# sydney-machine-learning/parallel-tempering-neural-net

Measured on AMD Instinct MI355X. Metric: MCMC samples/sec (all replicas) + swap-accept rate; Sunspot 64-replica FNN, higher is better.
Workload: dtype f32

## Files before the change

### parallel-tempering-neural-net_amd/csrc/ptnn_dev_pack.hpp

```cpp

constexpr int PK_WAVES = 8, PK_SWEEP_WAVES = 2, PK_FWD_WAVES = 4;
__host__ __device__ constexpr int pack_slots(int nred) { return PK_SWEEP_WAVES * (WAVE >> nred); }

__host__ __device__ inline size_t pack_slot_floats(int PS) { return 2 * (size_t)PS; }
__host__ __device__ inline size_t pack_ring_floats(int PS, int nslots) { return (size_t)2 * nslots * ((size_t)PS + 4); }
__host__ __device__ inline size_t pack_lds_floats(int Nall, int IPY, int PS, int H, int FWS, int nslots) {
    return (size_t)(Nall + 2) * IPY + 4 * (size_t)PS + MAX_WAVES * 8 + (size_t)nslots * SL_COUNT +
           (size_t)nslots * pack_slot_floats(PS) + pack_ring_floats(PS, nslots) + (size_t)PK_WAVES * fw_floats(H, FWS);
}
constexpr int PK_MULTI_MAXG = 4;
__host__ __device__ inline size_t pack_multi_lds_floats(int Nall, int IPY, int PS, int H, int FWS, int nslots) {
    return pack_lds_floats(Nall, IPY, PS, H, FWS, nslots) + pack_ring_floats(PS, (PK_MULTI_MAXG - 1) * nslots) + 2 * (size_t)PS + SL_COUNT + 8;
}

template <int TASK, int I, int O, int PK_NRED, bool MULTI = false>
__device__ __forceinline__ void segment_pack_body(const SegParams& p, const SegDyn& dyn, const int step_begin, const int n_steps) {
    constexpr int PK_NG = WAVE >> PK_NRED, PK_SLOTS = pack_slots(PK_NRED);
    extern __shared__ __attribute__((aligned(16))) float smem[];
    const int G = MULTI ? p.G : 1;
    const int lb = MULTI ? xcd_block(G) : (int)blockIdx.x;
    const int r = MULTI ? lb / G : lb, grp = MULTI ? lb - r * G : 0;
    const int KT = G * PK_SLOTS, s0 = grp * PK_SLOTS;
    const int gid = p.first_global + r;
    const int tid = threadIdx.x, nthr = blockDim.x;
    const int wave = tid >> 6, lane = tid & 63;
    const int Nall = p.Ntr + p.Nte;
    const int P = p.P, PS = p.PS, H = p.H;
    float* q = smem;
    float* xy = q; q += (Nall + 2) * p.IPY;
    float* w_cur = q; q += PS;
    float* w_gd = q; q += PS;
    float* rec_w = q; q += PS;
    float* rec_alt = q; q += PS;
    float* red = q; q += MAX_WAVES * 8;
    float* slots = q; q += PK_SLOTS * SL_COUNT;
    const size_t SLF = pack_slot_floats(PS);
    float* sl0 = q; q += PK_SLOTS * SLF;
    constexpr int RING = (MULTI ? 2 * PK_MULTI_MAXG : 2) * PK_SLOTS;
    float* ring_n = q; q += (size_t)RING * PS;
    float* ring_s = q; q += (size_t)RING * 4;
    float* my_fw = q + (size_t)wave * fw_floats(H, p.FWS);
    q += (size_t)PK_WAVES * fw_floats(H, p.FWS);
    float* win_v = q; q += MULTI ? 2 * (size_t)PS : 0;
    float* win_s = q; q += MULTI ? SL_COUNT : 0;
    float* gverd = q;
    granule_t* const xv = MULTI ? p.xverdict + (size_t)r * 2 * MAX_SLOTS : nullptr;
    granule_t* const xsl = MULTI ? p.xslots + (size_t)r * 2 * MAX_SLOTS * SL_COUNT : nullptr;
    granule_t* const xwv = MULTI ? p.xw + (size_t)r * 2 * G * 2 * PS : nullptr;
    unsigned epoch = dyn.epoch_base;
    int xpar = 0;
    bool failed = false;
    auto s_prop = [&](int s_) { return sl0 + (size_t)s_ * SLF; };
    auto s_pgd = [&](int s_) { return sl0 + (size_t)s_ * SLF + PS; };

    {
        const float4* src = reinterpret_cast<const float4*>(p.data);
        float4* dst = reinterpret_cast<float4*>(xy);
        for (int e = tid; e < ((Nall + 2) * p.IPY) >> 2; e += nthr) dst[e] = src[e];
    }
    float* gw = dyn.w_state + (size_t)r * PS;
    for (int j = tid; j < PS; j += nthr) {
        w_cur[j] = gw[j];
        rec_w[j] = p.rec_w[(size_t)r * PS + j];
        w_gd[j] = dyn.gd_w[(size_t)r * PS + j];
    }
    __syncthreads();

    const float T = uni_f(p.temps[r]);
    float eta = (TASK == TASK_REG) ? uni_f(w_cur[P]) : 0.0f;
    float* sf = p.st_f + (size_t)r * SF_COUNT;
    int* si = p.st_i + (size_t)r * SI_COUNT;
    float lik, prior_cur, tau_eta_last, rec_rmse_tr, rec_rmse_te, rec_acc_tr, rec_acc_te;
    int nacc, gd_valid, lg_count, lg_acc;
    if (step_begin == 0) {
        lg_acc = 0;
        if (wave == 0) {
            chain_startup<TASK, I, O, true>(p, xy, w_cur, my_fw, red, T, eta, lik, prior_cur);
            if (lane == 0) { red[0] = eta; red[1] = lik; red[2] = prior_cur; }
        }
        __syncthreads();
        eta = uni_f(red[0]); lik = uni_f(red[1]); prior_cur = uni_f(red[2]);
        tau_eta_last = eta;
        rec_rmse_tr = rec_rmse_te = rec_acc_tr = rec_acc_te = 0.f;
        nacc = 0; gd_valid = 0; lg_count = 0;
        __syncthreads();
    } else {
        lik = uni_f(sf[SF_LIK]); prior_cur = uni_f(sf[SF_PRIOR]); tau_eta_last = uni_f(sf[SF_TAU_LAST]);
        rec_rmse_tr = uni_f(sf[SF_REC_RMSE_TR]); rec_rmse_te = uni_f(sf[SF_REC_RMSE_TE]);
        rec_acc_tr = uni_f(sf[SF_REC_ACC_TR]); rec_acc_te = uni_f(sf[SF_REC_ACC_TE]);
        nacc = uni_i(si[SI_NACC]); gd_valid = uni_i(dyn.gd_valid[r]); lg_count = uni_i(si[SI_LG_COUNT]); lg_acc = uni_i(si[SI_LG_ACC]);
    }

    PTNN_DIAG(pack_begin);
    const size_t trow = (size_t)r * p.trace_cap;
    const int end = step_begin + n_steps;
    const bool sweeping = p.use_lg != 0;
    const int nwaves = nthr >> 6;
    const int ev_n = sweeping ? (nwaves == PK_WAVES ? PK_FWD_WAVES : 2) : nwaves;
    const int ev_i = !sweeping ? wave : ((wave & 3) >= 2 ? (wave & 1) + ((wave >> 2) << 1) : -1);
    int i = step_begin;
    int tpos0 = (step_begin + 1) % p.trace_cap;
    const float inv_PW = 1.0f / (float)p.PW;
    const int nq1 = ((P + 3) >> 2) + 1;
    auto fill_ring = [&](int lo, int hi, int wi, int nw) {
        if (nq1 <= WAVE) {
            const int per_pass = WAVE / nq1, ls = lane / nq1, q_ = lane - ls * nq1;
            for (int sb = lo + wi * per_pass; sb < hi; sb += nw * per_pass) {
                const int j = sb + ls;
                if (ls < per_pass && j < hi) {
                    const int slot = j % RING;
                    const bool sc = (q_ == nq1 - 1);
                    uint32_t x[4];
                    philox4x32_10(sc ? 0u : (uint32_t)q_, (uint32_t)j, p.noise_shared ? 0u : (uint32_t)gid, sc ? STREAM_STEP : STREAM_WNOISE,
                                  p.seed_lo, p.seed_hi, x);
                    float n0, n1, n2, n3;
                    box_muller(x[0], x[1], n0, n1);
                    box_muller(x[2], x[3], n2, n3);
                    if (sc) { float* sc_ = ring_s + slot * 4; sc_[0] = u23(x[0]); sc_[1] = u23(x[1]); sc_[2] = n2; }
                    else *reinterpret_cast<float4*>(ring_n + (size_t)slot * PS + 4 * q_) = make_float4(n0, n1, n2, n3);
                }
            }
        } else {
            for (int j = lo + wi; j < hi; j += nw) tape_step<true>(p, gid, j, ring_n + (size_t)(j % RING) * PS, ring_s + (j % RING) * 4);
        }
    };
    fill_ring(step_begin, step_begin + RING, wave, nwaves);
    int ring_hi = step_begin + RING;
    bool xcd_local = false;
    if constexpr (MULTI) {
        if (p.xcd_granules) xcd_local = xcd_handshake(xv + 32, G, grp, dyn.epoch_base, gverd);
    }
    __syncthreads();
    persist_cptr const pp = dyn.pp;
    const bool swap_inside = MULTI && pp->swap_inside != 0;
    const int si_ = pp->si;
    auto next_handoff = [&](int cur) {
        if (TASK == TASK_REG) { const int c1 = cur > 1 ? cur : 1; return ((c1 + si_ - 1) / si_) * si_; }
        return ((cur + si_) / si_) * si_ - 1;
    };
    int ho_next = swap_inside ? next_handoff(step_begin) : 0x7fffffff;
    int nx = 0;
    while (i < end && !failed) {
        if (MULTI) { epoch += 1; }
        if (i == p.switch_step) {
            if (wave == 0) {
                build_fw<I, O, true>(w_cur, my_fw, H, p.FWS);
                gsync<true>();
                const EvalSums sc = eval_rows<TASK, I, O, true>(my_fw, xy, p.IPY, p.FWS, H, p.Ntr, Nall, nullptr);
                float l2, r1, r2, a1, a2;
                finish_eval<TASK>(sc, p.Ntr, p.Nte, tau_eta_last, l2, r1, r2, a1, a2);
                if (lane == 0) red[0] = l2;
            }
            __syncthreads();
            lik = uni_f(red[0]);
            __syncthreads();
        }
        int kt = min(KT, end - i);
        if (p.switch_step > i) kt = min(kt, p.switch_step - i);
        if (swap_inside && ho_next >= i) kt = min(kt, ho_next - i + 1);
        const int k = MULTI ? max(0, min(PK_SLOTS, kt - s0)) : kt;
        PTNN_DIAG(count_round);
        STAMP(0);
        if (sweeping && !gd_valid) {
            if (wave == 0) sgd_sweep_dispatch<TASK, I, O>(w_cur, w_gd, xy, p.data, p.Ntr, H, p.lr);
            gd_valid = 1;
            __syncthreads();
        }
        const int rpos0 = (i + s0) % RING;
        auto s_noise = [&](int s_) { int e_ = rpos0 + s_; if (e_ >= RING) e_ -= RING; return ring_n + (size_t)e_ * PS; };
        auto s_scal = [&](int s_) { int e_ = rpos0 + s_; if (e_ >= RING) e_ -= RING; return ring_s + e_ * 4; };
        STAMP(1);
        STAMP(2);
        if (sweeping && wave < PK_SWEEP_WAVES) {
            const int ng = min(PK_NG, k - wave * PK_NG);
            if (ng > 0) {
                SweepProposals pp;
                pp.noise = ring_n; pp.scal = ring_s; pp.w_cur = w_cur; pp.w_gd = w_gd;
                pp.pos0 = rpos0 + wave * PK_NG; if (pp.pos0 >= RING) pp.pos0 -= RING;
                pp.ring = RING; pp.nstride = PS; pp.step_w = p.step_w; pp.l_prob = p.l_prob; pp.use_lg = 1;
                sgd_sweep<TASK, I, O, PK_NRED, true>(nullptr, s_pgd(wave * PK_NG), xy, p.data, p.Ntr, H, p.lr, ng, (int)SLF, &pp);
            }
        }
        STAMP(3);
        PTNN_DIAG(pack_eval_begin);
        if (ev_i >= 0) {
            for (int s_ = ev_i; s_ < k; s_ += ev_n) {
                const int j = i + s0 + s_;
                const float adapttemp = (p.switch_step >= 0 && j >= p.switch_step) ? 1.0f : T;
                const float* sc_ = s_scal(s_);
                const bool lg = sweeping && (sc_[0] < p.l_prob);
                float eta_pro = eta;
                if (TASK == TASK_REG) eta_pro = fmaf(p.step_eta, sc_[2], eta);
                {
                    const float* nz = s_noise(s_);
                    const float* base = lg ? w_gd : w_cur;
                    float* pr = s_prop(s_);
                    for (int e = lane; e < P; e += WAVE) pr[e] = fmaf(p.step_w, nz[e], base[e]);
                }
                gsync<true>();
                build_fw<I, O, true>(s_prop(s_), my_fw, H, p.FWS);
                gsync<true>();
                const EvalSums es = eval_rows<TASK, I, O, true>(my_fw, xy, p.IPY, p.FWS, H, p.Ntr, Nall, nullptr);
                float ll, rm_tr, rm_te, ac_tr, ac_te;
                finish_eval<TASK, true>(es, p.Ntr, p.Nte, eta_pro, ll, rm_tr, rm_te, ac_tr, ac_te);
                const float ssq = block_sumsq<true>(s_prop(s_), P, nullptr);
                const float prior_prop = prior_value<TASK>(p, ssq, eta_pro);
                const float d2 = lg ? block_sumsq<true>(s_noise(s_), P, nullptr) : 0.0f;
                if (lane == 0) {
                    float* sl = slots + s_ * SL_COUNT;
                    sl[SL_LIKPROP] = ll / adapttemp; sl[SL_PRIORPROP] = prior_prop; sl[SL_ETAPRO] = eta_pro;
                    sl[SL_RM_TR] = rm_tr; sl[SL_RM_TE] = rm_te; sl[SL_AC_TR] = ac_tr; sl[SL_AC_TE] = ac_te;
                    sl[SL_ADAPT] = adapttemp; sl[SL_LG] = lg ? 1.0f : 0.0f; sl[SL_D2] = d2;
                }
                gsync<true>();
            }
            fill_ring(ring_hi, i + RING, ev_i, ev_n);
        }
        ring_hi = i + RING;
        PTNN_DIAG(pack_eval_end);
        __syncthreads();
        STAMP(4);
        {
            const int s_ = wave * (WAVE / 16) + (lane >> 4), l16 = lane & 15;
            const bool on = s_ < k;
            float* sl = slots + (on ? s_ : 0) * SL_COUNT;
            float diff_prop = 0.0f;
            if (sweeping && wave < 4) {
                const float* pg = s_pgd(on ? s_ : 0);
                float r1[4];
#pragma unroll
                for (int c = 0; c < 4; ++c) {
                    float a1 = 0.0f;
                    for (int e = 16 * c + l16; e < P; e += WAVE) {
                        const float d = w_cur[e] - pg[e];
                        a1 = fmaf(d, d, a1);
                    }
                    r1[c] = (16 * c < P) ? group_allsum<4>(a1) : 0.0f;
                }
                const float d1 = (r1[0] + r1[1]) + (r1[2] + r1[3]);
                if (sl[SL_LG] != 0.0f) diff_prop = langevin_ratio(d1, sl[SL_D2], p.step_w, sl[SL_ADAPT]);
            }
            const float logalpha = (sl[SL_LIKPROP] - lik) + (sl[SL_PRIORPROP] - prior_cur) + diff_prop;
            const float mh = (logalpha != logalpha) ? 1.0f : fminf(1.0f, expf_fast(logalpha));
            if (on && l16 == 0) { sl[SL_ACCEPT] = (s_scal(s_)[1] < mh) ? 1.0f : 0.0f; sl[SL_LOGALPHA] = logalpha; }
        }
        __syncthreads();
        STAMP(5);
        const bool f_acc = (lane < k) && (slots[lane * SL_COUNT + SL_ACCEPT] != 0.0f);
        const unsigned long long bal_acc = __ballot(f_acc);
        const int ml = bal_acc ? (__ffsll((long long)bal_acc) - 1) : -1;
        int m = (ml >= 0) ? s0 + ml : kt;
        const float* sm = slots + (ml >= 0 ? ml : 0) * SL_COUNT;
        const float* wacc = s_prop(ml >= 0 ? ml : 0);
        if constexpr (MULTI) {
            granule_t* const xv_r = xv + (size_t)xpar * MAX_SLOTS;
            auto gstore = [&](granule_t* g_, float v_) { if (xcd_local) granule_store_xcd(g_, epoch, v_); else granule_store(g_, epoch, v_); };
            auto gwait = [&](const granule_t* g_, float& v_) { return xcd_local ? granule_wait_xcd(g_, epoch, v_) : granule_wait(g_, epoch, v_); };
            if (tid == 0) gstore(xv_r + grp, (float)ml);
            if (ml >= 0) {
                if (tid < SL_COUNT) gstore(xsl + ((size_t)xpar * MAX_SLOTS + grp) * SL_COUNT + tid, sm[tid]);
                granule_t* const xo = xwv + ((size_t)xpar * G + grp) * 2 * PS;
                for (int e = tid; e < 2 * PS; e += nthr) gstore(xo + e, wacc[e]);
            }
            if (tid < G) {
                float v = 0.0f;
                if (!gwait(xv_r + tid, v)) v = -2.0f;
                gverd[tid] = v;
            }
            __syncthreads();
            int win = -1;
            m = kt;
            for (int g_ = 0; g_ < G; ++g_) {
                const float v = gverd[g_];
                if (v == -2.0f) failed = true;
                const int cand = (v >= 0.0f) ? g_ * PK_SLOTS + (int)v : kt;
                if (cand < m) { m = cand; win = g_; }
            }
            if (failed) break;
            if (win >= 0 && win != grp) {
                bool ok = true;
                if (tid < SL_COUNT) {
                    float v;
                    ok = gwait(xsl + ((size_t)xpar * MAX_SLOTS + win) * SL_COUNT + tid, v);
                    win_s[tid] = v;
                }
                const granule_t* const xi = xwv + ((size_t)xpar * G + win) * 2 * PS;
                for (int e = tid; e < 2 * PS; e += nthr) {
                    float v;
                    ok = gwait(xi + e, v) && ok;
                    win_v[e] = v;
                }
                failed = __syncthreads_or(ok ? 0 : 1) != 0;
                if (failed) break;
                sm = win_s; wacc = win_v;
            }
            xpar ^= 1;
        }
        const int ncommit = (m < kt) ? m + 1 : kt;
        const int nloc = max(0, min(k, ncommit - s0));
        for (int item = tid; item < nloc * p.PW; item += nthr) {
            const int s_ = (int)(((float)item + 0.5f) * inv_PW), e = item - s_ * p.PW;
            int tp = tpos0 + s0 + s_;
            if (tp >= p.trace_cap) tp -= p.trace_cap;
            p.tr_pos_w[(trow + (size_t)tp) * (size_t)p.PW + e] = (e < P) ? ((s0 + s_ == m) ? s_prop(s_) : rec_w)[e] : 0.0f;
        }
        if (tid < nloc) {
            const int s_ = tid;
            const bool acc_me = (s0 + s_ == m);
            const float* sl = slots + s_ * SL_COUNT;
            int tp = tpos0 + s0 + s_;
            if (tp >= p.trace_cap) tp -= p.trace_cap;
            const size_t tpos = trow + (size_t)tp;
            store_trace_row(p.tr_scal + tpos * TR_COUNT, (TASK == TASK_REG) ? sl[SL_LIKPROP] : sl[SL_LIKPROP] * sl[SL_ADAPT],
                            acc_me ? sl[SL_RM_TR] : rec_rmse_tr, acc_me ? sl[SL_RM_TE] : rec_rmse_te,
                            acc_me ? sl[SL_AC_TR] : rec_acc_tr, acc_me ? sl[SL_AC_TE] : rec_acc_te, nacc, sl[SL_LOGALPHA]);
        }
        if constexpr (MULTI) {
            const int e_ = (i + lane) % RING;
            const bool f_lg = sweeping && (lane < ncommit) && (ring_s[e_ * 4] < p.l_prob);
            lg_count += __popcll(__ballot(f_lg));
            if (TASK == TASK_REG) tau_eta_last = uni_f(fmaf(p.step_eta, ring_s[((i + ncommit - 1) % RING) * 4 + 2], eta));
        } else {
            const bool f_lg = (lane < k) && (slots[lane * SL_COUNT + SL_LG] != 0.0f);
            const unsigned long long bal_lg = __ballot(f_lg);
            lg_count += __popcll(bal_lg & ((1ull << ncommit) - 1ull));
            if (TASK == TASK_REG) tau_eta_last = uni_f(slots[(ncommit - 1) * SL_COUNT + SL_ETAPRO]);
        }
        if (m < kt) {
            nacc += 1;
            lik = uni_f(sm[SL_LIKPROP]); prior_cur = uni_f(sm[SL_PRIORPROP]); eta = uni_f(sm[SL_ETAPRO]);
            rec_rmse_tr = uni_f(sm[SL_RM_TR]); rec_rmse_te = uni_f(sm[SL_RM_TE]);
            rec_acc_tr = uni_f(sm[SL_AC_TR]); rec_acc_te = uni_f(sm[SL_AC_TE]);
            lg_acc += (sm[SL_LG] != 0.0f) ? 1 : 0;
            gd_valid = sweeping ? 1 : 0;
            for (int e = tid; e < P; e += nthr) {
                const float v = wacc[e];
                w_cur[e] = v; rec_alt[e] = v;
                if (sweeping) w_gd[e] = wacc[PS + e];
            }
            float* t_ = rec_w; rec_w = rec_alt; rec_alt = t_;
        }
        __syncthreads();
        i += ncommit;
        tpos0 += ncommit;
        if (tpos0 >= p.trace_cap) tpos0 -= p.trace_cap;
        STAMP(6);
        if constexpr (MULTI) {
            if (swap_inside && i == ho_next + 1 && ho_next < end) {
                const int Rg = pp->sp.R, ROW = 2 * PS + 8;
                const unsigned xtag = dyn.epoch_base + (unsigned)nx + 1u;
                granule_t* const xl = p.xswap + (size_t)(nx & 1) * swap_xchg_granules(Rg, ROW);
                granule_t* const xst = xl + ((Rg + 7) & ~7);
                granule_t* const xsb = xst + (size_t)Rg * ROW + (size_t)gid * (ROW + 8);
                auto gstore = [&](granule_t* g_, float v_) { if (xcd_local) granule_store_xcd(g_, xtag, v_); else granule_store(g_, xtag, v_); };
                auto gwait = [&](const granule_t* g_, float& v_) { return xcd_local ? granule_wait_xcd(g_, xtag, v_) : granule_wait(g_, xtag, v_); };
                auto row_value = [&](int j) { return (j < PS) ? ((j == P) ? eta : ((j < P) ? w_cur[j] : 0.0f)) : ((j < 2 * PS) ? w_gd[j - PS] : ((j == 2 * PS) ? (gd_valid ? 1.0f : 0.0f) : 0.0f)); };
                auto row_take = [&](int j, float v) { if (j < PS) w_cur[j] = v; else if (j < 2 * PS) w_gd[j - PS] = v; else if (j == 2 * PS) red[1] = v; };
                bool ok = true;
                bool moved = false;
                if (grp == 0) {
                    if (tid == 0) granule_store(xl + gid, xtag, (TASK == TASK_REG) ? lik * T : lik);
                    for (int j = tid; j <= 2 * PS; j += nthr) granule_store(xst + (size_t)gid * ROW + j, xtag, row_value(j));
                    float* const sL = sl0;
                    float* const sU = sl0 + Rg;
                    int* const sSrc = reinterpret_cast<int*>(sl0 + 2 * Rg);
                    for (int k_ = tid; k_ < Rg; k_ += nthr) { float v = 0.0f; ok = granule_wait(xl + k_, xtag, v) && ok; sL[k_] = v; }
                    if (__syncthreads_or(ok ? 0 : 1)) { failed = true; break; }
#if defined(__HIP_DEVICE_COMPILE__)
                    const SwapParams sp = pp->sp;
#else
                    const SwapParams sp{};
#endif
                    const int round = pp->round0 + nx;
                    const int nsw = cascade_lds(sp, round, sL, sU, sSrc, true);
                    const int src = sSrc[gid];
                    if (gid == sp.first_global) {
                        if (sp.src_log && round < sp.log_capacity)
                            for (int k_ = tid; k_ < Rg; k_ += nthr) sp.src_log[(size_t)round * Rg + k_] = sSrc[k_];
                        if (tid == 0) { sp.counters[0] += nsw; sp.counters[1] += Rg - 1; }
                    }
                    __syncthreads();
                    moved = src != gid;
                    if (moved) {
                        for (int j = tid; j <= 2 * PS; j += nthr) { float v = 0.0f; ok = granule_wait(xst + (size_t)src * ROW + j, xtag, v) && ok; row_take(j, v); }
                        if (__syncthreads_or(ok ? 0 : 1)) { failed = true; break; }
                        for (int j = tid; j <= 2 * PS; j += nthr) gstore(xsb + 8 + j, (j == 2 * PS) ? red[1] : ((j < PS) ? w_cur[j] : w_gd[j - PS]));
                    }
                    if (tid == 0) gstore(xsb, moved ? 1.0f : 0.0f);
                } else {
                    if (tid == 0) { float mv = 0.0f; ok = gwait(xsb, mv); red[0] = mv; }
                    if (__syncthreads_or(ok ? 0 : 1)) { failed = true; break; }
                    moved = red[0] != 0.0f;
                    if (moved) {
                        for (int j = tid; j <= 2 * PS; j += nthr) { float v = 0.0f; ok = gwait(xsb + 8 + j, v) && ok; row_take(j, v); }
                        if (__syncthreads_or(ok ? 0 : 1)) { failed = true; break; }
                    }
                }
                __syncthreads();
                if (moved) {
                    if (TASK == TASK_REG) eta = uni_f(w_cur[P]);
                    gd_valid = (uni_f(red[1]) != 0.0f) ? 1 : 0;
                }
                __syncthreads();
                nx += 1;
                ho_next = next_handoff(i);
            }
        }
    }
    PTNN_DIAG(pack_flush);

    if (failed) {
        if (tid == 0) atomicAdd(p.error_flag, 1);
        return;
    }
    if (grp != 0) return;
    const int fl_end = (pp->flip0 + nx) & 1;
    float* const gw_end = swap_inside ? pp->state[fl_end] + (size_t)r * PS : gw;
    float* const gd_end = swap_inside ? pp->gd[fl_end] + (size_t)r * PS : dyn.gd_w + (size_t)r * PS;
    int* const gdv_end = swap_inside ? pp->gd_valid[fl_end] : dyn.gd_valid;
    for (int j = tid; j < PS; j += nthr) {
        gw_end[j] = (j == P) ? eta : w_cur[j];
        p.rec_w[(size_t)r * PS + j] = rec_w[j];
        gd_end[j] = w_gd[j];
    }
    if (tid == 0) {
        sf[SF_LIK] = lik; sf[SF_PRIOR] = prior_cur; sf[SF_TAU_LAST] = tau_eta_last;
        sf[SF_REC_RMSE_TR] = rec_rmse_tr; sf[SF_REC_RMSE_TE] = rec_rmse_te;
        sf[SF_REC_ACC_TR] = rec_acc_tr; sf[SF_REC_ACC_TE] = rec_acc_te;
        si[SI_NACC] = nacc; gdv_end[r] = gd_valid; si[SI_LG_COUNT] = lg_count; si[SI_LG_ACC] = lg_acc;
        p.L_handoff[gid] = (TASK == TASK_REG) ? lik * T : lik;
        p.L_final[gid] = lik;
        post_raw(p, gid, lik, prior_cur, T, step_begin + n_steps - 1);
    }
}
```

### parallel-tempering-neural-net_amd/csrc/ptnn_dev_spec.hpp

```cpp

enum { SL_ACCEPT = 0, SL_LIKPROP, SL_PRIORPROP, SL_ETAPRO, SL_RM_TR, SL_RM_TE, SL_AC_TR, SL_AC_TE, SL_LG, SL_ADAPT, SL_LOGALPHA, SL_D2, SL_COUNT = 16 };
constexpr int MAX_SLOTS = 64;
constexpr unsigned SPIN_LIMIT = 1u << 22;

__host__ __device__ inline size_t spec_wave_floats(int PS, int H, int FWS) { return 3 * (size_t)PS + fw_floats(H, FWS) + 8; }
__host__ __device__ inline size_t spec_lds_floats(int Nall, int IPY, int PS, int H, int FWS, int NW, int G) {
    return (size_t)(Nall + 2) * IPY + 3 * (size_t)PS + MAX_WAVES * 8 + 32 + (size_t)NW * G * SL_COUNT + (size_t)NW * spec_wave_floats(PS, H, FWS);
}

typedef unsigned long long granule_t;
__device__ __forceinline__ void granule_store(granule_t* g, unsigned epoch, float v) {
    __hip_atomic_store(g, ((granule_t)epoch << 32) | (granule_t)__builtin_bit_cast(unsigned, v), __ATOMIC_RELAXED,
                       __HIP_MEMORY_SCOPE_AGENT);
}
__device__ __forceinline__ bool granule_wait(const granule_t* g, unsigned epoch, float& v) {
    for (unsigned spins = 0; spins < SPIN_LIMIT; ++spins) {
        const granule_t x = __hip_atomic_load(g, __ATOMIC_RELAXED, __HIP_MEMORY_SCOPE_AGENT);
        if ((unsigned)(x >> 32) == epoch) { v = __builtin_bit_cast(float, (unsigned)x); return true; }
        __builtin_amdgcn_s_sleep(2);
    }
    return false;
}
__device__ __forceinline__ int xcc_id() {
    int x;
    asm volatile("s_getreg_b32 %0, hwreg(HW_REG_XCC_ID)" : "=s"(x));
    return x & 0xf;
}
__device__ __forceinline__ void granule_store_xcd(granule_t* g, unsigned epoch, float v) {
    const granule_t x = ((granule_t)epoch << 32) | (granule_t)__builtin_bit_cast(unsigned, v);
    asm volatile("global_store_dwordx2 %0, %1, off" ::"v"(g), "v"(x) : "memory");
}
__device__ __forceinline__ bool granule_wait_xcd(const granule_t* g, unsigned epoch, float& v, unsigned limit = SPIN_LIMIT) {
    for (unsigned spins = 0; spins < limit; ++spins) {
        granule_t x;
        asm volatile("global_load_dwordx2 %0, %1, off nt\n\ts_waitcnt vmcnt(0)" : "=v"(x) : "v"(g) : "memory");
        if ((unsigned)(x >> 32) == epoch) { v = __builtin_bit_cast(float, (unsigned)x); return true; }
        __builtin_amdgcn_s_sleep(1);
    }
    return false;
}
constexpr unsigned XCD_HANDSHAKE_SPINS = 1u << 13;
__device__ __forceinline__ bool xcd_handshake_strided(granule_t* ids, int stride, int G, int grp, unsigned tag, float* tmp) {
    const int my_xcc = xcc_id();
    if (threadIdx.x == 0) granule_store(ids + (size_t)grp * stride, tag, (float)my_xcc);
    if ((int)threadIdx.x < G) {
        float v = -1.0f;
        if (!granule_wait_xcd(ids + (size_t)threadIdx.x * stride, tag, v, XCD_HANDSHAKE_SPINS)) v = -2.0f;
        tmp[threadIdx.x] = v;
    }
    __syncthreads();
    bool same = true;
    for (int g_ = 0; g_ < G; ++g_) same = same && (tmp[g_] == (float)my_xcc);
    __syncthreads();
    return same;
}
__device__ __forceinline__ bool xcd_handshake(granule_t* ids, int G, int grp, unsigned tag, float* tmp) {
    return xcd_handshake_strided(ids, 1, G, grp, tag, tmp);
}


__device__ __forceinline__ int xcd_block(int G) {
    const int b = blockIdx.x, nb = gridDim.x;
#if defined(PTNN_NO_XCD_MAP)
    return b;
#else
    return (G > 1 && (nb & 7) == 0 && ((nb >> 3) % G) == 0) ? (b & 7) * (nb >> 3) + (b >> 3) : b;
#endif
}

struct SwapParams {
    int R, Rl, first_global, PS;
    uint32_t seed_lo, seed_hi;
    const float* L;
    const float* cur;
    float* next;
    const float* gd_cur;
    float* gd_next;
    const int* gd_valid_cur;
    int* gd_valid_next;
    int* src_out;
    long long* counters;
    int* src_log;
    int log_capacity;
    int rule, canonical;
    const float* L_raw;
    const float* prior_post;
    const float* temps_global;
    float* st_f;
    float* xchg;
    int XS;
    int L_stride;
    int label_mode;
    const int* label_cur;
    const int* slot_cur;
    int* label_next;
    int* slot_next;
    float* temps_local;
    int* progress;
    float* lad_hist;
    double* lad_s;
    float* lad_acc;
    float* lad_out;
    int lad_A, lad_acc_cap;
    double lad_kappa0, lad_t0;
};
__host__ __device__ inline int xchg_row_floats(int PS) { return (2 * PS + 4 + 3) & ~3; }

__device__ __forceinline__ int cascade_lds(const SwapParams& sp, int round, float* sL, float* sU, int* sSrc, bool have_L = false) {
    const int R = sp.R;
    for (int k = threadIdx.x; k < R; k += blockDim.x) {
        if (!have_L) sL[k] = sp.L[(size_t)(sp.label_mode ? sp.slot_cur[k] : k) * sp.L_stride];
        if (k < R - 1) {
            uint32_t x[4];
            philox4x32_10((uint32_t)k, (uint32_t)round, 0u, STREAM_SWAP, sp.seed_lo, sp.seed_hi, x);
            sU[k] = (sp.rule == 1) ? u23(x[0]) : logf_fast(2.0f * u23(x[0]));
        }
    }
    __syncthreads();
    if (sp.rule == 1) {
        for (int k = threadIdx.x; k < R; k += blockDim.x) sSrc[k] = k;
        if (threadIdx.x == 0) sSrc[R] = 0;
        __syncthreads();
        for (int k = (round & 1) + 2 * threadIdx.x; k < R - 1; k += 2 * blockDim.x) {
            const int s0 = sp.label_mode ? sp.slot_cur[k] : k, s1 = sp.label_mode ? sp.slot_cur[k + 1] : k + 1;
            const float d = (1.0f / sp.temps_global[k] - 1.0f / sp.temps_global[k + 1]) *
                            (sp.L_raw[(size_t)s1 * sp.L_stride] - sp.L_raw[(size_t)s0 * sp.L_stride]);
            const float pr = (d != d) ? 1.0f : fminf(1.0f, expf_fast(fminf(d, 80.0f)));
            if (sU[k] < pr) { sSrc[k] = k + 1; sSrc[k + 1] = k; atomicAdd(&sSrc[R], 1); }
        }
        __syncthreads();
        return sSrc[R];
    }
    if (threadIdx.x < WAVE) {
        const int lane = threadIdx.x;
        int c = 0, nsw = 0;
        float Lc = sL[0];
        for (int k0 = 0; k0 < R - 1; k0 += WAVE) {
            const int k = k0 + lane;
            const bool valid = k < R - 1;
            const float Ln = valid ? sL[k + 1] : 0.0f;
            const float tk = valid ? sU[k] : 0.0f;
            unsigned long long todo = __ballot(valid);
            unsigned long long swapped = 0ull;
            while (todo) {
                float d = Ln - Lc;
                d = (d < 709.0f) ? d : 709.0f;
                const unsigned long long fail = __ballot(!(tk < d)) & todo;
                if (!fail) { swapped |= todo; break; }
                const int j = __ffsll((long long)fail) - 1;
                swapped |= todo & ((1ull << j) - 1ull);
                if (lane == j) sSrc[k] = c;
                c = k0 + j + 1;
                Lc = __shfl(Ln, j);
                todo &= (j == 63) ? 0ull : ~((2ull << j) - 1ull);
            }
            if (valid && ((swapped >> lane) & 1ull)) sSrc[k] = k + 1;
            nsw += __popcll(swapped);
        }
        if (lane == 0) { sSrc[R - 1] = c; sSrc[R] = nsw; }
    }
    __syncthreads();
    return sSrc[R];
}

struct PersistParams {
    int end;
    int swap_inside;
    int task, si;
    int round0;
    int flip0, lflip0;
    int nblocks;
    unsigned* barrier;
    float* state[2];
    float* gd[2];
    int* gd_valid[2];
    int* label[2];
    int* slot_of[2];
    SwapParams sp;
};

__device__ __forceinline__ persist_cptr persist_args() {
    constexpr size_t off = (sizeof(SegParams) + alignof(PersistParams) - 1) & ~(alignof(PersistParams) - 1);
    unsigned long long a = (unsigned long long)(uintptr_t)__builtin_amdgcn_kernarg_segment_ptr() + off;
    asm volatile("" : "+s"(a));
    return (persist_cptr)(uintptr_t)a;
}

typedef __attribute__((address_space(4))) const SegParams* seg_cptr;
__device__ __forceinline__ seg_cptr seg_args() {
    unsigned long long a = (unsigned long long)(uintptr_t)__builtin_amdgcn_kernarg_segment_ptr();
    asm volatile("" : "+s"(a));
    return (seg_cptr)(uintptr_t)a;
}

__host__ __device__ inline size_t swap_xchg_granules(int R, int row) { return (size_t)((R + 7) & ~7) + (size_t)R * row + (size_t)R * (row + 8); }

template <int TASK, int I, int O>
__device__ __forceinline__ void segment_spec_body(const SegParams& p, const SegDyn& dyn, const int step_begin, const int n_steps) {
    extern __shared__ __attribute__((aligned(16))) float smem[];
    PTNN_DIAG(spec_entry);
    const int G = p.G;
    const int lb = xcd_block(G);
    const int r = lb / G, grp = lb - r * G;
    const int gid = p.first_global + r;
    const int tid = threadIdx.x, nthr = blockDim.x;
    const int wave = tid >> 6, lane = tid & 63, NW = nthr >> 6;
    const int K = NW * G;
    const int sidx = grp * NW + wave;
    const int Nall = p.Ntr + p.Nte;
    const int P = p.P, PS = p.PS, H = p.H;
    float* q = smem;
    float* xy = q; q += (Nall + 2) * p.IPY;
    float* w_cur = q; q += PS;
    float* w_gd = q; q += PS;
    float* rec_w = q; q += PS;
    float* red = q; q += MAX_WAVES * 8;
    unsigned* pready = reinterpret_cast<unsigned*>(q); unsigned* fclaim = pready + MAX_WAVES; unsigned* fdone = fclaim + MAX_WAVES; q += 32;
    float* slots = q; q += K * SL_COUNT;
    const size_t wfl = spec_wave_floats(PS, H, p.FWS);
    float* priv0 = q;
    float* mine = priv0 + (size_t)wave * wfl;
    float* my_prop = mine;
    float* my_pgd = mine + PS;
    float* my_noise = mine + 2 * PS;
    float* my_fw = mine + 3 * PS;
    float* my_scal = my_fw + fw_floats(H, p.FWS);
    granule_t* xs = p.xslots + (size_t)r * 2 * MAX_SLOTS * SL_COUNT;
    granule_t* xw = p.xw + (size_t)r * 2 * MAX_SLOTS * 2 * PS;
    granule_t* xv = p.xverdict + (size_t)r * 2 * MAX_SLOTS;

    {
        const float4* src = reinterpret_cast<const float4*>(p.data);
        float4* dst = reinterpret_cast<float4*>(xy);
        for (int e = tid; e < ((Nall + 2) * p.IPY) >> 2; e += nthr) dst[e] = src[e];
    }
    float* gw = dyn.w_state + (size_t)r * PS;
    for (int j = tid; j < PS; j += nthr) {
        w_cur[j] = gw[j];
        rec_w[j] = p.rec_w[(size_t)r * PS + j];
        w_gd[j] = dyn.gd_w[(size_t)r * PS + j];
    }
    if (tid < 3 * MAX_WAVES) pready[tid] = 0u;
    __syncthreads();

    const float T = uni_f(p.temps[r]);
    float eta = (TASK == TASK_REG) ? uni_f(w_cur[P]) : 0.0f;
    float* sf = p.st_f + (size_t)r * SF_COUNT;
    int* si = p.st_i + (size_t)r * SI_COUNT;
    float lik, prior_cur, tau_eta_last, rec_rmse_tr, rec_rmse_te, rec_acc_tr, rec_acc_te;
    int nacc, gd_valid, lg_count, lg_acc;
    if (step_begin == 0) {
        lg_acc = 0;
        if (wave == 0) {
            chain_startup<TASK, I, O, true>(p, xy, w_cur, my_fw, red, T, eta, lik, prior_cur);
            if (lane == 0) { red[0] = eta; red[1] = lik; red[2] = prior_cur; }
        }
        __syncthreads();
        eta = uni_f(red[0]); lik = uni_f(red[1]); prior_cur = uni_f(red[2]);
        tau_eta_last = eta;
        rec_rmse_tr = rec_rmse_te = rec_acc_tr = rec_acc_te = 0.f;
        nacc = 0; gd_valid = 0; lg_count = 0;
        __syncthreads();
    } else {
        lik = uni_f(sf[SF_LIK]); prior_cur = uni_f(sf[SF_PRIOR]); tau_eta_last = uni_f(sf[SF_TAU_LAST]);
        rec_rmse_tr = uni_f(sf[SF_REC_RMSE_TR]); rec_rmse_te = uni_f(sf[SF_REC_RMSE_TE]);
        rec_acc_tr = uni_f(sf[SF_REC_ACC_TR]); rec_acc_te = uni_f(sf[SF_REC_ACC_TE]);
        nacc = uni_i(si[SI_NACC]); gd_valid = uni_i(dyn.gd_valid[r]); lg_count = uni_i(si[SI_LG_COUNT]); lg_acc = uni_i(si[SI_LG_ACC]);
    }

    PTNN_DIAG(spec_begin);
    const size_t trow = (size_t)r * p.trace_cap;
    const int end = step_begin + n_steps;
    int i = step_begin;
    unsigned epoch = dyn.epoch_base;
    int par = 0;
    bool failed = false;
    STAMP(0);
    while (i < end) {
        epoch += 1;
        PTNN_DIAG(count_round);
        if (i == p.switch_step) {
            if (wave == 0) {
                build_fw<I, O, true>(w_cur, my_fw, H, p.FWS);
                gsync<true>();
                const EvalSums sc = eval_rows<TASK, I, O, true>(my_fw, xy, p.IPY, p.FWS, H, p.Ntr, Nall, nullptr);
                float l2, r1, r2, a1, a2;
                finish_eval<TASK>(sc, p.Ntr, p.Nte, tau_eta_last, l2, r1, r2, a1, a2);
                if (lane == 0) red[0] = l2;
            }
            __syncthreads();
            lik = uni_f(red[0]);
            __syncthreads();
        }
        int k = min(K, end - i);
        if (p.switch_step > i) k = min(k, p.switch_step - i);
        const int j = i + sidx;
        const bool active = sidx < k;
        bool lg = false;
        float u = 0.f, n_eta = 0.f;
        if (active) {
            tape_step<true>(p, gid, j, my_noise, my_scal);
            gsync<true>();
            const float lx = my_scal[0];
            u = my_scal[1];
            n_eta = my_scal[2];
            lg = p.use_lg && (lx < p.l_prob);
        }
        STAMP(1);
        if (p.use_lg && !gd_valid) {
            if (wave == 0) sgd_sweep_dispatch<TASK, I, O>(w_cur, w_gd, xy, p.data, p.Ntr, H, p.lr);
            gd_valid = 1;
            __syncthreads();
        }
        float* sl = slots + sidx * SL_COUNT;
        bool acc_mine = false;
        STAMP(2);
        auto forward_of = [&](const float* prop, float eta_x, float adapt_x, float& lik_prop, float& prior_prop, float& rm_tr,
                              float& rm_te, float& ac_tr, float& ac_te) {
            build_fw<I, O, true>(prop, my_fw, H, p.FWS);
            gsync<true>();
            const EvalSums es = eval_rows<TASK, I, O, true>(my_fw, xy, p.IPY, p.FWS, H, p.Ntr, Nall, nullptr);
            float ll;
            finish_eval<TASK, true>(es, p.Ntr, p.Nte, eta_x, ll, rm_tr, rm_te, ac_tr, ac_te);
            lik_prop = ll / adapt_x;
            const float ssq = block_sumsq<true>(prop, P, nullptr);
            prior_prop = prior_value<TASK>(p, ssq, eta_x);
        };
        if (active) {
            const float adapttemp = (p.switch_step >= 0 && j >= p.switch_step) ? 1.0f : T;
            float diff_prop = 0.0f;
            float eta_pro = eta;
            if (TASK == TASK_REG) eta_pro = fmaf(p.step_eta, n_eta, eta);
            float lik_prop = 0.f, prior_prop = 0.f, rm_tr = 0.f, rm_te = 0.f, ac_tr = 0.f, ac_te = 0.f;
            bool have_forward = false;
            if (lg) {
                for (int e = lane; e < P; e += WAVE) my_prop[e] = fmaf(p.step_w, my_noise[e], w_gd[e]);
                if (lane == 0) { sl[SL_ETAPRO] = eta_pro; sl[SL_ADAPT] = adapttemp; }
                gsync<true>();
                __builtin_amdgcn_fence(__ATOMIC_RELEASE, "workgroup");
                if (lane == 0) __hip_atomic_store(pready + wave, epoch, __ATOMIC_RELAXED, __HIP_MEMORY_SCOPE_WORKGROUP);
                sgd_sweep_dispatch<TASK, I, O>(my_prop, my_pgd, xy, p.data, p.Ntr, H, p.lr);
                gsync<true>();
                const float d1 = block_sumsq_diff<true>(w_cur, my_pgd, P, nullptr);
                const float d2 = block_sumsq<true>(my_noise, P, nullptr);
                diff_prop = langevin_ratio(d1, d2, p.step_w, adapttemp);
                unsigned prev = 0u;
                if (lane == 0) prev = __hip_atomic_exchange(fclaim + wave, epoch, __ATOMIC_RELAXED, __HIP_MEMORY_SCOPE_WORKGROUP);
                prev = (unsigned)uni_i((int)prev);
                if (prev == epoch) {
                    bool done = false;
                    for (unsigned spins = 0; spins < (1u << 20) && !done; ++spins) {
                        done = uni_i((int)__hip_atomic_load(fdone + wave, __ATOMIC_RELAXED, __HIP_MEMORY_SCOPE_WORKGROUP)) == (int)epoch;
                        if (!done) __builtin_amdgcn_s_sleep(1);
                    }
                    if (done) {
                        __builtin_amdgcn_fence(__ATOMIC_ACQUIRE, "workgroup");
                        lik_prop = uni_f(sl[SL_LIKPROP]); prior_prop = uni_f(sl[SL_PRIORPROP]);
                        rm_tr = uni_f(sl[SL_RM_TR]); rm_te = uni_f(sl[SL_RM_TE]); ac_tr = uni_f(sl[SL_AC_TR]); ac_te = uni_f(sl[SL_AC_TE]);
                        have_forward = true;
                    }
                }
            } else {
                for (int e = lane; e < P; e += WAVE) my_prop[e] = fmaf(p.step_w, my_noise[e], w_cur[e]);
                gsync<true>();
            }
            STAMP(3);
            if (!have_forward) forward_of(my_prop, eta_pro, adapttemp, lik_prop, prior_prop, rm_tr, rm_te, ac_tr, ac_te);
            const float logalpha = (lik_prop - lik) + (prior_prop - prior_cur) + diff_prop;
            const float mh = (logalpha != logalpha) ? 1.0f : fminf(1.0f, expf_fast(logalpha));
            acc_mine = u < mh;
            STAMP(4);
            if (p.use_lg && !lg && acc_mine) {
                sgd_sweep_dispatch<TASK, I, O>(my_prop, my_pgd, xy, p.data, p.Ntr, H, p.lr);
                gsync<true>();
            }
            if (lane == 0) {
                sl[SL_ACCEPT] = acc_mine ? 1.0f : 0.0f;
                sl[SL_LIKPROP] = lik_prop; sl[SL_PRIORPROP] = prior_prop; sl[SL_ETAPRO] = eta_pro;
                sl[SL_RM_TR] = rm_tr; sl[SL_RM_TE] = rm_te; sl[SL_AC_TR] = ac_tr; sl[SL_AC_TE] = ac_te;
                sl[SL_LG] = lg ? 1.0f : 0.0f; sl[SL_ADAPT] = adapttemp; sl[SL_LOGALPHA] = logalpha;
            }
            if (G > 1 && acc_mine) {
                gsync<true>();
                if (lane < SL_COUNT) granule_store(xs + ((size_t)par * MAX_SLOTS + sidx) * SL_COUNT + lane, epoch, sl[lane]);
                granule_t* xo = xw + ((size_t)par * MAX_SLOTS + sidx) * 2 * PS;
                for (int e = lane; e < 2 * PS; e += WAVE) granule_store(xo + e, epoch, mine[e]);
            }
        }
        if (G > 1 && lane == 0) granule_store(xv + (size_t)par * MAX_SLOTS + sidx, epoch, (active && acc_mine) ? 1.0f : 0.0f);
        STAMP(5);
        if (p.use_lg) {
            for (int t_ = 0; t_ < NW; ++t_) {
                if (t_ == wave) continue;
                const bool ready = uni_i((int)__hip_atomic_load(pready + t_, __ATOMIC_RELAXED, __HIP_MEMORY_SCOPE_WORKGROUP)) == (int)epoch;
                if (!ready) continue;
                unsigned prev = epoch;
                if (lane == 0) prev = __hip_atomic_exchange(fclaim + t_, epoch, __ATOMIC_RELAXED, __HIP_MEMORY_SCOPE_WORKGROUP);
                prev = (unsigned)uni_i((int)prev);
                if (prev == epoch) continue;
                __builtin_amdgcn_fence(__ATOMIC_ACQUIRE, "workgroup");
                float* slt = slots + (grp * NW + t_) * SL_COUNT;
                float lp, pp, r1, r2, a1, a2;
                forward_of(priv0 + (size_t)t_ * wfl, uni_f(slt[SL_ETAPRO]), uni_f(slt[SL_ADAPT]), lp, pp, r1, r2, a1, a2);
                if (lane == 0) {
                    slt[SL_LIKPROP] = lp; slt[SL_PRIORPROP] = pp; slt[SL_RM_TR] = r1; slt[SL_RM_TE] = r2; slt[SL_AC_TR] = a1; slt[SL_AC_TE] = a2;
                }
                gsync<true>();
                __builtin_amdgcn_fence(__ATOMIC_RELEASE, "workgroup");
                if (lane == 0) __hip_atomic_store(fdone + t_, epoch, __ATOMIC_RELAXED, __HIP_MEMORY_SCOPE_WORKGROUP);
            }
        }
        __syncthreads();
        STAMP(6);
        if (G > 1) {
            bool ok = true;
            if (tid < K && tid / NW != grp) {
                const int s_ = tid;
                float v = 0.0f;
                ok = granule_wait(xv + (size_t)par * MAX_SLOTS + s_, epoch, v);
                if (s_ < k) {
                    uint32_t x[4];
                    philox4x32_10(0u, (uint32_t)(i + s_), p.noise_shared ? 0u : (uint32_t)gid, STREAM_STEP, p.seed_lo, p.seed_hi, x);
                    float n2, n3;
                    box_muller(x[2], x[3], n2, n3);
                    float* fs = slots + s_ * SL_COUNT;
                    fs[SL_ACCEPT] = v;
                    fs[SL_LG] = (p.use_lg && u23(x[0]) < p.l_prob) ? 1.0f : 0.0f;
                    fs[SL_ETAPRO] = (TASK == TASK_REG) ? fmaf(p.step_eta, n2, eta) : eta;
                }
            }
            if (__syncthreads_or(ok ? 0 : 1)) { failed = true; break; }
        }
        STAMP(7);
        const bool my_flag_acc = (lane < k) && (slots[lane * SL_COUNT + SL_ACCEPT] != 0.0f);
        const bool my_flag_lg = (lane < k) && (slots[lane * SL_COUNT + SL_LG] != 0.0f);
        const unsigned long long bal_acc = __ballot(my_flag_acc), bal_lg = __ballot(my_flag_lg);
        const int m = bal_acc ? (__ffsll((long long)bal_acc) - 1) : k;
        const int ncommit = (m < k) ? m + 1 : k;
        if (sidx < ncommit) {
            const bool acc_me = (sidx == m);
            const float* srcw = acc_me ? my_prop : rec_w;
            const size_t tpos = trow + (size_t)((j + 1) % p.trace_cap);
            float* prow = p.tr_pos_w + tpos * (size_t)p.PW;
            for (int e = lane; e < p.PW; e += WAVE) prow[e] = (e < P) ? srcw[e] : 0.0f;
            if (lane == 0) {
                store_trace_row(p.tr_scal + tpos * TR_COUNT, (TASK == TASK_REG) ? sl[SL_LIKPROP] : sl[SL_LIKPROP] * sl[SL_ADAPT],
                                acc_me ? sl[SL_RM_TR] : rec_rmse_tr, acc_me ? sl[SL_RM_TE] : rec_rmse_te,
                                acc_me ? sl[SL_AC_TR] : rec_acc_tr, acc_me ? sl[SL_AC_TE] : rec_acc_te,
                                nacc , sl[SL_LOGALPHA]);
            }
        }
        lg_count += __popcll(bal_lg & ((ncommit >= 64) ? ~0ull : ((1ull << ncommit) - 1ull)));
        if (TASK == TASK_REG) tau_eta_last = uni_f(slots[(ncommit - 1) * SL_COUNT + SL_ETAPRO]);
        __syncthreads();
        if (m < k) {
            const int owner = m / NW;
            bool ok = true;
            if (G > 1 && owner != grp) {
                if (tid < SL_COUNT) {
                    float v = 0.0f;
                    ok = granule_wait(xs + ((size_t)par * MAX_SLOTS + m) * SL_COUNT + tid, epoch, v);
                    slots[m * SL_COUNT + tid] = v;
                }
                if (__syncthreads_or(ok ? 0 : 1)) { failed = true; break; }
            }
            const float* sm = slots + m * SL_COUNT;
            nacc += 1;
            lik = uni_f(sm[SL_LIKPROP]); prior_cur = uni_f(sm[SL_PRIORPROP]); eta = uni_f(sm[SL_ETAPRO]);
            rec_rmse_tr = uni_f(sm[SL_RM_TR]); rec_rmse_te = uni_f(sm[SL_RM_TE]);
            rec_acc_tr = uni_f(sm[SL_AC_TR]); rec_acc_te = uni_f(sm[SL_AC_TE]);
            gd_valid = p.use_lg ? 1 : 0;
            lg_acc += (sm[SL_LG] != 0.0f) ? 1 : 0;
            if (owner == grp) {
                const float* wacc = priv0 + (size_t)(m - grp * NW) * wfl;
                for (int e = tid; e < P; e += nthr) {
                    const float v = wacc[e];
                    w_cur[e] = v; rec_w[e] = v;
                    if (p.use_lg) w_gd[e] = wacc[PS + e];
                }
            } else {
                const granule_t* xo = xw + ((size_t)par * MAX_SLOTS + m) * 2 * PS;
                for (int e = tid; e < P; e += nthr) {
                    float v = 0.f, gv = 0.f;
                    ok = granule_wait(xo + e, epoch, v) && ok;
                    if (p.use_lg) ok = granule_wait(xo + PS + e, epoch, gv) && ok;
                    w_cur[e] = v; rec_w[e] = v;
                    if (p.use_lg) w_gd[e] = gv;
                }
            }
            if (G > 1 && __syncthreads_or(ok ? 0 : 1)) { failed = true; break; }
        }
        __syncthreads();
        i += ncommit;
        par ^= 1;
        STAMP(8);
    }
    PTNN_DIAG(spec_flush);

    if (failed) {
        if (tid == 0) atomicAdd(p.error_flag, 1);
        return;
    }
    if (grp == 0) {
        for (int j = tid; j < PS; j += nthr) {
            gw[j] = (j == P) ? eta : w_cur[j];
            p.rec_w[(size_t)r * PS + j] = rec_w[j];
            dyn.gd_w[(size_t)r * PS + j] = w_gd[j];
        }
        if (tid == 0) {
            sf[SF_LIK] = lik; sf[SF_PRIOR] = prior_cur; sf[SF_TAU_LAST] = tau_eta_last;
            sf[SF_REC_RMSE_TR] = rec_rmse_tr; sf[SF_REC_RMSE_TE] = rec_rmse_te;
            sf[SF_REC_ACC_TR] = rec_acc_tr; sf[SF_REC_ACC_TE] = rec_acc_te;
            si[SI_NACC] = nacc; dyn.gd_valid[r] = gd_valid; si[SI_LG_COUNT] = lg_count; si[SI_LG_ACC] = lg_acc;
            p.L_handoff[gid] = (TASK == TASK_REG) ? lik * T : lik;
            p.L_final[gid] = lik;
            post_raw(p, gid, lik, prior_cur, T, step_begin + n_steps - 1);
        }
    }
}
```

Measured before the change: 15.65 million.

## Double-buffer pack slots to defer trace writes and drop an accept barrier

In the single-block pack path, slot metadata and proposal buffers become double-buffered. Trace-row writes for a round are deferred and issued by the eval waves during the next round's evaluation, overlapping global stores with compute. The Langevin distance d1 is now computed in the sweep waves right after the SGD sweep and stored in a new slot field. This lets the accept decision run with one lane per slot and no extra __syncthreads. The cost is more LDS for the doubled buffers and more state carried across iterations, with a final flush after the loop.

```diff
diff --git a/parallel-tempering-neural-net_amd/csrc/ptnn_dev_pack.hpp b/parallel-tempering-neural-net_amd/csrc/ptnn_dev_pack.hpp
--- a/parallel-tempering-neural-net_amd/csrc/ptnn_dev_pack.hpp
+++ b/parallel-tempering-neural-net_amd/csrc/ptnn_dev_pack.hpp
@@ -4,13 +4,16 @@
 
 __host__ __device__ inline size_t pack_slot_floats(int PS) { return 2 * (size_t)PS; }
 __host__ __device__ inline size_t pack_ring_floats(int PS, int nslots) { return (size_t)2 * nslots * ((size_t)PS + 4); }
+__host__ __device__ inline size_t pack_lds_floats_n(int Nall, int IPY, int PS, int H, int FWS, int nslots, int nbuf) {
+    return (size_t)(Nall + 2) * IPY + 4 * (size_t)PS + MAX_WAVES * 8 + (size_t)nbuf * nslots * SL_COUNT +
+           (size_t)nbuf * nslots * pack_slot_floats(PS) + pack_ring_floats(PS, nslots) + (size_t)PK_WAVES * fw_floats(H, FWS);
+}
 __host__ __device__ inline size_t pack_lds_floats(int Nall, int IPY, int PS, int H, int FWS, int nslots) {
-    return (size_t)(Nall + 2) * IPY + 4 * (size_t)PS + MAX_WAVES * 8 + (size_t)nslots * SL_COUNT +
-           (size_t)nslots * pack_slot_floats(PS) + pack_ring_floats(PS, nslots) + (size_t)PK_WAVES * fw_floats(H, FWS);
+    return pack_lds_floats_n(Nall, IPY, PS, H, FWS, nslots, 2);
 }
 constexpr int PK_MULTI_MAXG = 4;
 __host__ __device__ inline size_t pack_multi_lds_floats(int Nall, int IPY, int PS, int H, int FWS, int nslots) {
-    return pack_lds_floats(Nall, IPY, PS, H, FWS, nslots) + pack_ring_floats(PS, (PK_MULTI_MAXG - 1) * nslots) + 2 * (size_t)PS + SL_COUNT + 8;
+    return pack_lds_floats_n(Nall, IPY, PS, H, FWS, nslots, 1) + pack_ring_floats(PS, (PK_MULTI_MAXG - 1) * nslots) + 2 * (size_t)PS + SL_COUNT + 8;
 }
 
 template <int TASK, int I, int O, int PK_NRED, bool MULTI = false>
@@ -33,9 +36,12 @@
     float* rec_w = q; q += PS;
     float* rec_alt = q; q += PS;
     float* red = q; q += MAX_WAVES * 8;
-    float* slots = q; q += PK_SLOTS * SL_COUNT;
+    constexpr int NBUF = MULTI ? 1 : 2;
+    float* const slots_b = q; q += NBUF * PK_SLOTS * SL_COUNT;
     const size_t SLF = pack_slot_floats(PS);
-    float* sl0 = q; q += PK_SLOTS * SLF;
+    float* const sl0_b = q; q += NBUF * PK_SLOTS * SLF;
+    float* slots = slots_b;
+    float* sl0 = sl0_b;
     constexpr int RING = (MULTI ? 2 * PK_MULTI_MAXG : 2) * PK_SLOTS;
     float* ring_n = q; q += (size_t)RING * PS;
     float* ring_s = q; q += (size_t)RING * 4;
@@ -101,6 +107,31 @@
     int i = step_begin;
     int tpos0 = (step_begin + 1) % p.trace_cap;
     const float inv_PW = 1.0f / (float)p.PW;
+    int par = 0, pd_n = 0, pd_m = 0, pd_tpos0 = 0, pd_nacc = 0;
+    bool pd_acc = false;
+    float pd_rmse_tr = 0.f, pd_rmse_te = 0.f, pd_acc_tr = 0.f, pd_acc_te = 0.f;
+    auto write_pending = [&](int t0, int nt) {
+        const float* const psl = slots_b + (size_t)(par ^ 1) * PK_SLOTS * SL_COUNT;
+        const float* const pv0 = sl0_b + (size_t)(par ^ 1) * PK_SLOTS * SLF;
+        const float* const prec = pd_acc ? rec_alt : rec_w;
+        for (int item = t0; item < pd_n * p.PW; item += nt) {
+            const int s_ = (int)(((float)item + 0.5f) * inv_PW), e = item - s_ * p.PW;
+            int tp = pd_tpos0 + s_;
+            if (tp >= p.trace_cap) tp -= p.trace_cap;
+            p.tr_pos_w[(trow + (size_t)tp) * (size_t)p.PW + e] = (e < P) ? ((s_ == pd_m) ? pv0 + (size_t)s_ * SLF : prec)[e] : 0.0f;
+        }
+        if (t0 < pd_n) {
+            const int s_ = t0;
+            const bool acc_me = (s_ == pd_m);
+            const float* sl = psl + s_ * SL_COUNT;
+            int tp = pd_tpos0 + s_;
+            if (tp >= p.trace_cap) tp -= p.trace_cap;
+            const size_t tpos = trow + (size_t)tp;
+            store_trace_row(p.tr_scal + tpos * TR_COUNT, (TASK == TASK_REG) ? sl[SL_LIKPROP] : sl[SL_LIKPROP] * sl[SL_ADAPT],
+                            acc_me ? sl[SL_RM_TR] : pd_rmse_tr, acc_me ? sl[SL_RM_TE] : pd_rmse_te,
+                            acc_me ? sl[SL_AC_TR] : pd_acc_tr, acc_me ? sl[SL_AC_TE] : pd_acc_te, pd_nacc, sl[SL_LOGALPHA]);
+        }
+    };
     const int nq1 = ((P + 3) >> 2) + 1;
     auto fill_ring = [&](int lo, int hi, int wi, int nw) {
         if (nq1 <= WAVE) {
@@ -142,6 +173,10 @@
     int nx = 0;
     while (i < end && !failed) {
         if (MULTI) { epoch += 1; }
+        if constexpr (!MULTI) {
+            slots = slots_b + (size_t)par * PK_SLOTS * SL_COUNT;
+            sl0 = sl0_b + (size_t)par * PK_SLOTS * SLF;
+        }
         if (i == p.switch_step) {
             if (wave == 0) {
                 build_fw<I, O, true>(w_cur, my_fw, H, p.FWS);
@@ -179,11 +214,36 @@
                 pp.pos0 = rpos0 + wave * PK_NG; if (pp.pos0 >= RING) pp.pos0 -= RING;
                 pp.ring = RING; pp.nstride = PS; pp.step_w = p.step_w; pp.l_prob = p.l_prob; pp.use_lg = 1;
                 sgd_sweep<TASK, I, O, PK_NRED, true>(nullptr, s_pgd(wave * PK_NG), xy, p.data, p.Ntr, H, p.lr, ng, (int)SLF, &pp);
+                if constexpr (!MULTI) {
+                    gsync<true>();
+                    const int l16 = lane & 15;
+                    for (int g0 = 0; g0 < ng; g0 += WAVE / 16) {
+                        const int g_ = g0 + (lane >> 4);
+                        const bool on = g_ < ng;
+                        const int s_ = wave * PK_NG + (on ? g_ : 0);
+                        const float* pg = s_pgd(s_);
+                        float r1[4];
+#pragma unroll
+                        for (int c = 0; c < 4; ++c) {
+                            float a1 = 0.0f;
+                            for (int e = 16 * c + l16; e < P; e += WAVE) {
+                                const float d = w_cur[e] - pg[e];
+                                a1 = fmaf(d, d, a1);
+                            }
+                            r1[c] = (16 * c < P) ? group_allsum<4>(a1) : 0.0f;
+                        }
+                        const float d1 = (r1[0] + r1[1]) + (r1[2] + r1[3]);
+                        if (on && l16 == 0) slots[s_ * SL_COUNT + SL_D1] = d1;
+                    }
+                }
             }
         }
         STAMP(3);
         PTNN_DIAG(pack_eval_begin);
         if (ev_i >= 0) {
+            if constexpr (!MULTI) {
+                if (pd_n > 0) write_pending(ev_i * WAVE + lane, ev_n * WAVE);
+            }
             for (int s_ = ev_i; s_ < k; s_ += ev_n) {
                 const int j = i + s0 + s_;
                 const float adapttemp = (p.switch_step >= 0 && j >= p.switch_step) ? 1.0f : T;
@@ -220,34 +280,48 @@
         PTNN_DIAG(pack_eval_end);
         __syncthreads();
         STAMP(4);
-        {
-            const int s_ = wave * (WAVE / 16) + (lane >> 4), l16 = lane & 15;
-            const bool on = s_ < k;
-            float* sl = slots + (on ? s_ : 0) * SL_COUNT;
+        unsigned long long bal_acc;
+        if constexpr (MULTI) {
+            {
+                const int s_ = wave * (WAVE / 16) + (lane >> 4), l16 = lane & 15;
+                const bool on = s_ < k;
+                float* sl = slots + (on ? s_ : 0) * SL_COUNT;
+                float diff_prop = 0.0f;
+                if (sweeping && wave < 4) {
+                    const float* pg = s_pgd(on ? s_ : 0);
+                    float r1[4];
+#pragma unroll
+                    for (int c = 0; c < 4; ++c) {
+                        float a1 = 0.0f;
+                        for (int e = 16 * c + l16; e < P; e += WAVE) {
+                            const float d = w_cur[e] - pg[e];
+                            a1 = fmaf(d, d, a1);
+                        }
+                        r1[c] = (16 * c < P) ? group_allsum<4>(a1) : 0.0f;
+                    }
+                    const float d1 = (r1[0] + r1[1]) + (r1[2] + r1[3]);
+                    if (sl[SL_LG] != 0.0f) diff_prop = langevin_ratio(d1, sl[SL_D2], p.step_w, sl[SL_ADAPT]);
+                }
+                const float logalpha = (sl[SL_LIKPROP] - lik) + (sl[SL_PRIORPROP] - prior_cur) + diff_prop;
+                const float mh = (logalpha != logalpha) ? 1.0f : fminf(1.0f, expf_fast(logalpha));
+                if (on && l16 == 0) { sl[SL_ACCEPT] = (s_scal(s_)[1] < mh) ? 1.0f : 0.0f; sl[SL_LOGALPHA] = logalpha; }
+            }
+            __syncthreads();
+            STAMP(5);
+            const bool f_acc = (lane < k) && (slots[lane * SL_COUNT + SL_ACCEPT] != 0.0f);
+            bal_acc = __ballot(f_acc);
+        } else {
+            const bool on = lane < k;
+            float* sl = slots + (on ? lane : 0) * SL_COUNT;
             float diff_prop = 0.0f;
-            if (sweeping && wave < 4) {
-                const float* pg = s_pgd(on ? s_ : 0);
-                float r1[4];
-#pragma unroll
-                for (int c = 0; c < 4; ++c) {
-                    float a1 = 0.0f;
-                    for (int e = 16 * c + l16; e < P; e += WAVE) {
-                        const float d = w_cur[e] - pg[e];
-                        a1 = fmaf(d, d, a1);
-                    }
-                    r1[c] = (16 * c < P) ? group_allsum<4>(a1) : 0.0f;
-                }
-                const float d1 = (r1[0] + r1[1]) + (r1[2] + r1[3]);
-                if (sl[SL_LG] != 0.0f) diff_prop = langevin_ratio(d1, sl[SL_D2], p.step_w, sl[SL_ADAPT]);
-            }
+            if (sweeping && sl[SL_LG] != 0.0f) diff_prop = langevin_ratio(sl[SL_D1], sl[SL_D2], p.step_w, sl[SL_ADAPT]);
             const float logalpha = (sl[SL_LIKPROP] - lik) + (sl[SL_PRIORPROP] - prior_cur) + diff_prop;
             const float mh = (logalpha != logalpha) ? 1.0f : fminf(1.0f, expf_fast(logalpha));
-            if (on && l16 == 0) { sl[SL_ACCEPT] = (s_scal(s_)[1] < mh) ? 1.0f : 0.0f; sl[SL_LOGALPHA] = logalpha; }
-        }
-        __syncthreads();
-        STAMP(5);
-        const bool f_acc = (lane < k) && (slots[lane * SL_COUNT + SL_ACCEPT] != 0.0f);
-        const unsigned long long bal_acc = __ballot(f_acc);
+            const bool f_acc = on && (s_scal(on ? lane : 0)[1] < mh);
+            if (on && wave == nwaves - 1) sl[SL_LOGALPHA] = logalpha;
+            STAMP(5);
+            bal_acc = __ballot(f_acc);
+        }
         const int ml = bal_acc ? (__ffsll((long long)bal_acc) - 1) : -1;
         int m = (ml >= 0) ? s0 + ml : kt;
         const float* sm = slots + (ml >= 0 ? ml : 0) * SL_COUNT;
@@ -298,22 +372,28 @@
         }
         const int ncommit = (m < kt) ? m + 1 : kt;
         const int nloc = max(0, min(k, ncommit - s0));
-        for (int item = tid; item < nloc * p.PW; item += nthr) {
-            const int s_ = (int)(((float)item + 0.5f) * inv_PW), e = item - s_ * p.PW;
-            int tp = tpos0 + s0 + s_;
-            if (tp >= p.trace_cap) tp -= p.trace_cap;
-            p.tr_pos_w[(trow + (size_t)tp) * (size_t)p.PW + e] = (e < P) ? ((s0 + s_ == m) ? s_prop(s_) : rec_w)[e] : 0.0f;
-        }
-        if (tid < nloc) {
-            const int s_ = tid;
-            const bool acc_me = (s0 + s_ == m);
-            const float* sl = slots + s_ * SL_COUNT;
-            int tp = tpos0 + s0 + s_;
-            if (tp >= p.trace_cap) tp -= p.trace_cap;
-            const size_t tpos = trow + (size_t)tp;
-            store_trace_row(p.tr_scal + tpos * TR_COUNT, (TASK == TASK_REG) ? sl[SL_LIKPROP] : sl[SL_LIKPROP] * sl[SL_ADAPT],
-                            acc_me ? sl[SL_RM_TR] : rec_rmse_tr, acc_me ? sl[SL_RM_TE] : rec_rmse_te,
-                            acc_me ? sl[SL_AC_TR] : rec_acc_tr, acc_me ? sl[SL_AC_TE] : rec_acc_te, nacc, sl[SL_LOGALPHA]);
+        if constexpr (MULTI) {
+            for (int item = tid; item < nloc * p.PW; item += nthr) {
+                const int s_ = (int)(((float)item + 0.5f) * inv_PW), e = item - s_ * p.PW;
+                int tp = tpos0 + s0 + s_;
+                if (tp >= p.trace_cap) tp -= p.trace_cap;
+                p.tr_pos_w[(trow + (size_t)tp) * (size_t)p.PW + e] = (e < P) ? ((s0 + s_ == m) ? s_prop(s_) : rec_w)[e] : 0.0f;
+            }
+            if (tid < nloc) {
+                const int s_ = tid;
+                const bool acc_me = (s0 + s_ == m);
+                const float* sl = slots + s_ * SL_COUNT;
+                int tp = tpos0 + s0 + s_;
+                if (tp >= p.trace_cap) tp -= p.trace_cap;
+                const size_t tpos = trow + (size_t)tp;
+                store_trace_row(p.tr_scal + tpos * TR_COUNT, (TASK == TASK_REG) ? sl[SL_LIKPROP] : sl[SL_LIKPROP] * sl[SL_ADAPT],
+                                acc_me ? sl[SL_RM_TR] : rec_rmse_tr, acc_me ? sl[SL_RM_TE] : rec_rmse_te,
+                                acc_me ? sl[SL_AC_TR] : rec_acc_tr, acc_me ? sl[SL_AC_TE] : rec_acc_te, nacc, sl[SL_LOGALPHA]);
+            }
+        } else {
+            pd_n = nloc; pd_m = m; pd_tpos0 = tpos0; pd_nacc = nacc; pd_acc = m < kt;
+            pd_rmse_tr = rec_rmse_tr; pd_rmse_te = rec_rmse_te; pd_acc_tr = rec_acc_tr; pd_acc_te = rec_acc_te;
+            par ^= 1;
         }
         if constexpr (MULTI) {
             const int e_ = (i + lane) % RING;
@@ -407,6 +487,9 @@
             }
         }
     }
+    if constexpr (!MULTI) {
+        if (pd_n > 0) write_pending(tid, nthr);
+    }
     PTNN_DIAG(pack_flush);
 
     if (failed) {
diff --git a/parallel-tempering-neural-net_amd/csrc/ptnn_dev_spec.hpp b/parallel-tempering-neural-net_amd/csrc/ptnn_dev_spec.hpp
--- a/parallel-tempering-neural-net_amd/csrc/ptnn_dev_spec.hpp
+++ b/parallel-tempering-neural-net_amd/csrc/ptnn_dev_spec.hpp
@@ -1,5 +1,5 @@
 
-enum { SL_ACCEPT = 0, SL_LIKPROP, SL_PRIORPROP, SL_ETAPRO, SL_RM_TR, SL_RM_TE, SL_AC_TR, SL_AC_TE, SL_LG, SL_ADAPT, SL_LOGALPHA, SL_D2, SL_COUNT = 16 };
+enum { SL_ACCEPT = 0, SL_LIKPROP, SL_PRIORPROP, SL_ETAPRO, SL_RM_TR, SL_RM_TE, SL_AC_TR, SL_AC_TE, SL_LG, SL_ADAPT, SL_LOGALPHA, SL_D2, SL_D1, SL_COUNT = 16 };
 constexpr int MAX_SLOTS = 64;
 constexpr unsigned SPIN_LIMIT = 1u << 22;
 
```

Result: slower. 15.32 million (-2.1%).
